# jjshoots/PyFlyt

Measured on AMD Instinct MI355X. Metric: env-steps/sec (whole node), QuadX-Hover batch=65536 per GPU, higher is better.
Workload: dtype f32

## Files before the change

pyflyt_amd/csrc/quadx_fast.hpp:

```cpp
#pragma once
#include <cstdlib>
#include <cstring>
#include <type_traits>

#include "../../include/pyflyt_amd.h"
#include "uav_device.hpp"
#include "uav_vehicles.hpp"
#include "quadx_control_d.hpp"
#include "shared_world.hpp"
#include "policy_mlp.hpp"

namespace pf {

struct QuadK {
  float dt, half_dt, gravity_z, vmax, inv_mass;
  float I[3], iI[3];
  float use_gyro;
  float bound_radius;
  float bound_radius0, slop;
  float margin;
  float brk, rd;
  float c_erp;
  int32_t c_all8;
  float box_h[3], plane_xy, plane_z;
// ... 1006 lines not shown
  const int op = FIXED ? (int)OP_STEP : op_arg;
  const uint8_t* const mask = FIXED ? nullptr : mask_arg;
  const int k_autoreset = FIXED ? (int)PF_AUTORESET_NEXT_STEP : K.autoreset;
  const int k_step_ratio = FIXED ? kQuadFixedRatio<TASK> : K.env_step_ratio;
  const bool k_quat = FIXED || K.angle_repr != 0;
  const bool k_sparse = !FIXED && K.task_sparse != 0;
  constexpr bool REKEY = TASK == PF_TASK_HOVER || TASK == PF_TASK_WAYPOINTS;
  constexpr bool SPARE = REKEY && !MODES && !SHARED && NOISE != PF_NOISE_INJECT;
  typedef QuadSpare Sp;
  constexpr bool GIVEN = ROLL == 2;
  constexpr int kMaxD = 13 + 4 + 4 + 16;
  constexpr int kSettleMax = 24;
  __shared__ __attribute__((aligned(16))) float tile_all[kQuadWPB * LPW * kMaxD];
  __shared__ __attribute__((aligned(16))) float sxi_all[kQuadWPB * 64 * kSettleMax];
  __shared__ int spos_all[kQuadWPB * 64];
  __shared__ float wpose_all[SHARED ? kQuadWPB * 64 * 8 : 1];
  __shared__ float wvel_all[SHARED ? kQuadWPB * 64 * kPairVelStride : 1];
  __shared__ uint32_t sctr_all[kQuadWPB * 64];
  __shared__ __attribute__((aligned(16))) float splds_all[(ROLLOUT && SPARE) ? kQuadWPB * 64 * 20 : 4];
  const int wid = kQuadWPB > 1 ? (int)(threadIdx.x >> 6) : 0;
  const int tid = kQuadWPB > 1 ? (int)(threadIdx.x & 63u) : (int)threadIdx.x;
  float* const tile = tile_all + wid * (LPW * kMaxD);
  float* const sxi = sxi_all + wid * (64 * kSettleMax);
  int* const spos = spos_all + wid * 64;
  uint32_t* const sctr = sctr_all + wid * 64;
  float* const wpose = wpose_all + (SHARED ? wid * 64 * 8 : 0);
  const int apw = SHARED ? K.apw : 1;
  const int wave_base = (blockIdx.x * kQuadWPB + wid) * LPW;
  if (kQuadWPB > 1 && wave_base >= n) return;
  const int lane = wave_base + tid;
  const bool valid = (tid < LPW) && (lane < n);
  const size_t li = valid ? (size_t)lane : (size_t)(n - 1);
  const size_t N = (size_t)n;
  const float4* Sin = reinterpret_cast<const float4*>(B.state);
  float4* Sout = reinterpret_cast<float4*>(B.state);
#ifdef PF_PHASE_TRACE
  unsigned long long pf_ts[kPhaseStamps];
  pf_ts[11] = __builtin_amdgcn_s_memrealtime();
#endif
  PF_STAMP(0);

  QuadHot V;
  constexpr bool DSTATE = MODES && !SHARED;
  QuadStateD SD;
  static_assert(LPW * kMaxD >= kContactSlotFloats, "the contact solver's LDS regions alias the observation tile: at least one worst-case region");
  V.cws = (lds_fptr)tile;
  V.cws_floats = LPW * kMaxD;
  if (SHARED) { V.wpose_ = wpose; V.wvel_ = wvel_all + wid * 64 * kPairVelStride; V.rec_ = tile; V.wtid = tid; V.wA = apw; }
  QuadCascT<typename std::conditional<DSTATE, double, float>::type> C;
  const pf_params_kptr Pk = uniform_params(Pfull);
  constexpr bool CALM = CR && !SHARED && !MODES && NOISE != PF_NOISE_INJECT;
  QuadKV KV{};
  if (CALM) KV = quadkv_from(K);
  float tgt[4][3];
  float new_dist, old_dist;
  int step_count, flags, n_left;
  uint32_t rng_ctr;
  f8 zn;
  uint32_t call0 = 0u;
  uint32_t rkw = 0u;
  bool sp_dirty = false;
  uint32_t reset_key_now = 0u;
  Sp spv{};
  float* const splds = splds_all + ((ROLLOUT && SPARE) ? (wid * 64 + tid) * 20 : 0);
  float4 a_pre = float4{0.f, 0.f, 0.f, 0.f};
  const float4 f4z = float4{0.f, 0.f, 0.f, 0.f};
  float4 cm0 = f4z, cm1 = f4z, cm2 = f4z, cm3 = f4z, cm4 = f4z, cm5 = f4z, cm6 = f4z, cm7 = f4z, cm8 = f4z, cm9 = f4z;
  {
    float4 gi = Sin[6 * N + li];
    float4 g0 = Sin[0 * N + li], g1 = Sin[1 * N + li], g2 = Sin[2 * N + li], g3 = Sin[3 * N + li], g4 = Sin[4 * N + li],
           g5 = Sin[5 * N + li];
    float4 gs7 = float4{0.f, 0.f, 0.f, 0.f};
    if (SPARE) gs7 = Sin[7 * N + li];
    if (SPARE) {
      typedef const uint32_t __attribute__((address_space(1))) * gu32ptr;
      uintptr_t ca = reinterpret_cast<uintptr_t>(launch_ctr + kCtrStride * blockIdx.x);
      asm volatile("" : "+v"(ca));
      call0 = *reinterpret_cast<gu32ptr>(ca);
    }
    if (ROLL == 0 && op == OP_STEP) a_pre = reinterpret_cast<const float4*>(B.actions)[li];
    float4 dl0 = float4{0.f, 0.f, 0.f, 0.f}, dl1 = dl0, dl2 = dl0, dl3 = dl0;
    float4 dl4 = dl0, dl5 = dl0;
    if (DSTATE) { dl0 = Sin[16 * N + li]; dl1 = Sin[17 * N + li]; dl2 = Sin[18 * N + li]; dl3 = Sin[19 * N + li]; dl4 = Sin[20 * N + li]; dl5 = Sin[21 * N + li]; }
    if (MODES) {
      cm0 = Sin[7 * N + li]; cm1 = Sin[8 * N + li]; cm2 = Sin[9 * N + li]; cm3 = Sin[10 * N + li]; cm4 = Sin[11 * N + li];
      if (DSTATE) { cm5 = Sin[22 * N + li]; cm6 = Sin[23 * N + li]; cm7 = Sin[24 * N + li]; cm8 = Sin[25 * N + li]; cm9 = Sin[26 * N + li]; }
    }
    if (CR && blockIdx.x < kRareTextPrefetchBlocks) rare_text_prefetch(tid);
    rng_ctr = (uint32_t)__float_as_int(gi.z);
    PF_STAMP(1);
    if (REKEY) {
      const bool in11 = MODES && K.mode > 0;
      const bool need_sp = SPARE || ROLLOUT || in11 || op == OP_RESET || k_autoreset == PF_AUTORESET_SAME_STEP ||
                           (__float_as_int(gi.y) & (PF_F_TERMINATED | PF_F_TRUNCATED)) != 0;
      if (need_sp) {
        const float4 gk = SPARE ? gs7 : (in11 ? cm4 : (MODES ? cm0 : Sin[(size_t)7 * N + li]));
        rkw = (uint32_t)__float_as_int(in11 ? gk.z : gk.w);
        if (SPARE && op == OP_RESET && mask == nullptr) rkw &= ~kSpareValid;
        if (SPARE) {
          spv.z = gk.x; spv.vz = gk.y; spv.thr = gk.z;
          if constexpr (ROLL == 3) {
            float4* r4 = reinterpret_cast<float4*>(splds);
            r4[0] = float4{spv.z, spv.vz, spv.thr, 0.0f};
            if (TASK == PF_TASK_WAYPOINTS) { r4[1] = Sin[8 * N + li]; r4[2] = Sin[9 * N + li]; r4[3] = Sin[10 * N + li]; r4[4] = Sin[11 * N + li]; }
          } else {
          if (TASK == PF_TASK_WAYPOINTS) { spv.t[0] = Sin[8 * N + li]; spv.t[1] = Sin[9 * N + li]; spv.t[2] = Sin[10 * N + li]; spv.t[3] = Sin[11 * N + li]; }
          if (ROLLOUT) {
            float4* r4 = reinterpret_cast<float4*>(splds);
            r4[0] = float4{spv.z, spv.vz, spv.thr, 0.0f};
            if (TASK == PF_TASK_WAYPOINTS) { r4[1] = spv.t[0]; r4[2] = spv.t[1]; r4[3] = spv.t[2]; r4[4] = spv.t[3]; }
          }
          }
        }
      }
    }
    if (NOISE == PF_NOISE_PHILOX) {
      if (op == OP_STEP) zn = normal8(philox4x32(K.seed_lo, K.seed_hi, (uint32_t)(lane0 + li), rng_ctr, 0u, 0u));
    }
    PF_STAMP(2);
    V.p = v3{g0.x, g0.y, g0.z}; new_dist = g0.w;
    V.q = quat{g1.x, g1.y, g1.z, g1.w};
    V.set_wv(v3{g2.w, g3.x, g3.y}, v3{g2.x, g2.y, g2.z});
    V.t01 = f2{g3.z, g3.w}; V.t23 = f2{g4.x, g4.y};
    V.I[0] = g4.z; V.I[1] = g4.w; V.I[2] = g5.x;
    V.E[0] = g5.y; V.E[1] = g5.z; V.E[2] = g5.w;
    if (DSTATE) {
      SD.p[0] = (double)g0.x + (double)dl0.x; SD.p[1] = (double)g0.y + (double)dl0.y; SD.p[2] = (double)g0.z + (double)dl0.z;
      SD.q[0] = (double)g1.x + (double)dl0.w; SD.q[1] = (double)g1.y + (double)dl1.x; SD.q[2] = (double)g1.z + (double)dl1.y; SD.q[3] = (double)g1.w + (double)dl1.z;
      SD.v[0] = (double)g2.x + (double)dl1.w; SD.v[1] = (double)g2.y + (double)dl2.x; SD.v[2] = (double)g2.z + (double)dl2.y;
      SD.w[0] = (double)g2.w + (double)dl2.z; SD.w[1] = (double)g3.x + (double)dl2.w; SD.w[2] = (double)g3.y + (double)dl3.x;
      SD.rI[0] = (double)g4.z + (double)dl4.x; SD.rI[1] = (double)g4.w + (double)dl4.y; SD.rI[2] = (double)g5.x + (double)dl4.z;
      SD.rE[0] = (double)g5.y + (double)dl4.w; SD.rE[1] = (double)g5.z + (double)dl5.x; SD.rE[2] = (double)g5.w + (double)dl5.y;
      SD.thr[0] = (double)g3.z + (double)dl3.y; SD.thr[1] = (double)g3.w + (double)dl3.z; SD.thr[2] = (double)g4.x + (double)dl3.w; SD.thr[3] = (double)g4.y + (double)dl5.z;
#pragma unroll
      for (int k = 0; k < 4; ++k) SD.pwm[k] = 0.05;
      SD.derive();
    }
    step_count = __float_as_int(gi.x); flags = __float_as_int(gi.y);
    n_left = __float_as_int(gi.w);
    if (TASK == PF_TASK_WAYPOINTS || TASK == PF_TASK_MA_HOVER) {
      float4 a = Sin[12 * N + li], b = Sin[13 * N + li], c = Sin[14 * N + li];
      tgt[0][0] = a.x; tgt[0][1] = a.y; tgt[0][2] = a.z; tgt[1][0] = a.w;
      tgt[1][1] = b.x; tgt[1][2] = b.y; tgt[2][0] = b.z; tgt[2][1] = b.w;
      tgt[2][2] = c.x; tgt[3][0] = c.y; tgt[3][1] = c.z; tgt[3][2] = c.w;
    }
  }
  old_dist = new_dist;
  if (MODES && K.mode > 0) {
    C.unpack(cm0, cm1, cm2, cm3, cm4, false);
    if constexpr (DSTATE) C.unpack(cm5, cm6, cm7, cm8, cm9, true);
  } else C.zero();
  float4 ma_past = float4{0.f, 0.f, 0.f, 0.f};
  if (TASK == PF_TASK_MA_HOVER) ma_past = Sin[15 * N + li];
  const bool kYaw = (TASK == PF_TASK_WAYPOINTS) && K.use_yaw != 0;
  float ytg[4] = {0.f, 0.f, 0.f, 0.f};
  float yaw_err0 = 0.0f;
  if (kYaw) { float4 y = Sin[15 * N + li]; ytg[0] = y.x; ytg[1] = y.y; ytg[2] = y.z; ytg[3] = y.w; }
  auto yaw_now = [&]() {
    if (__builtin_fabsf(V.R.m20) >= 0.99999f) return euler_from_quat(V.q).z;
    return fast_atan2(V.R.m10, V.R.m00);
  };
  auto wrap_pi = [](float e) {
    e = e > kPi ? e - 2.0f * kPi : e;
    return e < -kPi ? e + 2.0f * kPi : e;
  };
  V.contact_now = (flags & PF_F_CONTACT) != 0;
  V.contact_step = false;
  V.derive();
#ifdef PF_PHASE_TRACE
  asm volatile("" ::"v"(V.wb.x), "v"(V.vb.z));
#endif
  PF_STAMP(3);
  bool term = (flags & PF_F_TERMINATED) != 0, trunc = (flags & PF_F_TRUNCATED) != 0;

  bool active;
  if (op == OP_RESET) active = (mask == nullptr) || (mask[li] != 0);
  else active = true;
  active = active && valid;
  if (SHARED && op == OP_RESET) active = widen_to_world(active, tid, apw) && valid;

  float act0 = 0.f, act1 = 0.f, act2 = 0.f, act3 = 0.f;
  float reward = 0.0f;
  bool pop_pending = false;
  bool was_reset = false;
  const int D = (k_quat ? 13 : 12) + 8 + (TASK == PF_TASK_WAYPOINTS ? (kYaw ? 4 : 3) * K.num_targets : (TASK == PF_TASK_MA_HOVER ? 3 : 0));
  const int settle_ticks = K.settle_steps * 2;

  auto pop_target = [&]() {
#pragma unroll
    for (int k = 0; k < 3; ++k)
#pragma unroll
      for (int c = 0; c < 3; ++c) tgt[k][c] = tgt[k + 1][c];
    ytg[0] = ytg[1]; ytg[1] = ytg[2]; ytg[2] = ytg[3];
    n_left -= 1;
  };
  auto lds_sync = [&]() { lds_sync_wave(); };
  const bool coop_targets = (TASK == PF_TASK_WAYPOINTS) && !((NOISE == PF_NOISE_INJECT) && (B.u_targets != nullptr));
  auto prepare_reset_draws = [&](const bool reset_now, const uint32_t key) {
    const bool want_noise = NOISE == PF_NOISE_PHILOX;
    if (!want_noise && !coop_targets) return;
    const unsigned long long m = __ballot(reset_now);
    if (m == 0ull) return;
    const int r = __popcll(m);
    uint32_t seed_lo = K.seed_lo, seed_hi = K.seed_hi;
    asm volatile("" : "+s"(seed_lo), "+s"(seed_hi));
    if (reset_now) {
      spos[__popcll(m & ((1ull << tid) - 1ull))] = tid;
      sctr[tid] = key;
    }
    lds_sync();
    const int ncall = want_noise ? (settle_ticks + 7) >> 3 : 0;
    const int nt = K.num_targets, ntc = coop_targets ? (kYaw ? 4 : 3) : 0;
    const int per = ncall + ntc;
    float* const U = tile;
    float* const TG = tile + 64 * 16;
    for (int base = 0; base < r * per; base += 64) {
      const int j = base + tid;
      if (j < r * per) {
        const int which = j / per, c = j - which * per;
        const int src = spos[which];
// ... 218 lines not shown
            phi = B.u_targets[(size_t)(nt + i) * N + li] * (0.5f / kPi);
            dist = B.u_targets[(size_t)(2 * nt + i) * N + li];
          } else {
            theta = u(i);
            phi = u(nt + i);
            dist = fmaf(K.dome09m1, u(2 * nt + i), 1.0f);
          }
          float st, ct, sph, cph;
          sincos_turns(theta, st, ct);
          sincos_turns(phi, sph, cph);
          float zz = __builtin_fabsf(dist * cph);
          tgt[i][0] = dist * sph * ct; tgt[i][1] = dist * sph * st; tgt[i][2] = zz > K.min_height ? zz : K.min_height;
        }
      }
      }
      float dx = tgt[0][0] - V.p.x, dy = tgt[0][1] - V.p.y, dz = tgt[0][2] - V.p.z;
      old_dist = INFINITY;
      new_dist = fsqrt(fmaf(dx, dx, fmaf(dy, dy, dz * dz)));
      if (kYaw) yaw_err0 = __builtin_fabsf(wrap_pi(ytg[0] - yaw_now()));
    }
    rng_ctr += 1;
    if (REKEY) { rkw = rng_ctr & ~kSpareValid; sp_dirty = true; }
    was_reset = true;
  };
  auto make_spare = [&](const bool me, const uint32_t key, Sp& out) {
    prepare_reset_draws(me, key);
    if (me) {
      float z = K.start_pos[2], vz = 0.f, thr = 0.f, pw = 0.05f;
      settle_run(z, vz, thr, pw);
      out.z = z; out.vz = vz; out.thr = thr;
      if (TASK == PF_TASK_WAYPOINTS) {
        const float4* t4 = reinterpret_cast<const float4*>(tile + 64 * 16 + tid * 16);
#pragma unroll
        for (int i = 0; i < 4; ++i) out.t[i] = t4[i];
      }
    }
  };
  auto spare_get = [&]() -> Sp {
    if (!ROLLOUT) return spv;
    Sp x;
    const float4* r4 = reinterpret_cast<const float4*>(splds);
    const float4 a0 = r4[0];
    x.z = a0.x; x.vz = a0.y; x.thr = a0.z;
    if (TASK == PF_TASK_WAYPOINTS) { x.t[0] = r4[1]; x.t[1] = r4[2]; x.t[2] = r4[3]; x.t[3] = r4[4]; }
    return x;
  };
  auto spare_put = [&](const Sp& x) {
    if (!ROLLOUT) { spv = x; return; }
    float4* r4 = reinterpret_cast<float4*>(splds);
    r4[0] = float4{x.z, x.vz, x.thr, 0.0f};
    if (TASK == PF_TASK_WAYPOINTS) { r4[1] = x.t[0]; r4[2] = x.t[1]; r4[3] = x.t[2]; r4[4] = x.t[3]; }
  };
  auto do_resets = [&](const bool r) {
    const bool have = SPARE && r && (rkw & kSpareValid) != 0u;
    reset_key_now = REKEY ? (rkw & ~kSpareValid) : rng_ctr;
    prepare_reset_draws(r && !have, reset_key_now);
    if (!MODES || __any(r)) {
      if (r) {
        if (SPARE && __builtin_expect(have, 1)) reset_lane(true, spare_get());
        else reset_lane(false, Sp{});
      }
    }
  };
  auto refill_spares = [&](const bool now) {
    if (!SPARE || !now) return;
    const bool want = active && (rkw & kSpareValid) == 0u;
    if (!__any(want)) return;
    Sp g{};
    make_spare(want, rkw & ~kSpareValid, g);
    if (want) { spare_put(g); rkw |= kSpareValid; sp_dirty = true; }
  };
  auto write_obs_row = [&]() {
    float* row = tile + tid * D;
    float sarg = -V.R.m20;
    quat qe;
    v3 rpy;
    const float obs_yaw = kYaw ? yaw_now() : 0.0f;
    if (__builtin_fabsf(sarg) >= 0.99999f) {
      rpy = euler_from_quat(V.q);
      qe = quat_from_euler(rpy);
    } else {
      float ar = V.R.m21, br = V.R.m22;
      float ay = V.R.m10, by = V.R.m00;
      float hr = frsq(fmaf(ar, ar, br * br)), hy = frsq(fmaf(ay, ay, by * by));
      float cr, sr, cp, sp, cy, sy;
      half_angle(br * hr, ar * hr, cr, sr);
      half_angle(fsqrt((1.0f - sarg) * (1.0f + sarg)), sarg, cp, sp);
      half_angle(by * hy, ay * hy, cy, sy);
      quat t = quat_from_half_angles(cr, sr, cp, sp, cy, sy);
      float inv = frsq(fmaf(t.x, t.x, fmaf(t.y, t.y, fmaf(t.z, t.z, t.w * t.w))));
      qe = quat{t.x * inv, t.y * inv, t.z * inv, t.w * inv};
      if (!k_quat) rpy = v3{fast_atan2(ar, br), fast_asin(sarg), fast_atan2(ay, by)};
    }
    int k = 0;
    row[k++] = V.wb.x; row[k++] = V.wb.y; row[k++] = V.wb.z;
    if (k_quat) { row[k++] = qe.x; row[k++] = qe.y; row[k++] = qe.z; row[k++] = qe.w; }
    else { row[k++] = rpy.x; row[k++] = rpy.y; row[k++] = rpy.z; }
    row[k++] = V.vb.x; row[k++] = V.vb.y; row[k++] = V.vb.z;
    row[k++] = V.p.x; row[k++] = V.p.y; row[k++] = V.p.z;
    if (TASK == PF_TASK_MA_HOVER) {
      row[k++] = V.t01.x; row[k++] = V.t01.y; row[k++] = V.t23.x; row[k++] = V.t23.y;
      row[k++] = ma_past.x; row[k++] = ma_past.y; row[k++] = ma_past.z; row[k++] = ma_past.w;
      row[k++] = tgt[0][0]; row[k++] = tgt[0][1]; row[k++] = tgt[0][2];
    } else {
      row[k++] = act0; row[k++] = act1; row[k++] = act2; row[k++] = act3;
      row[k++] = V.t01.x; row[k++] = V.t01.y; row[k++] = V.t23.x; row[k++] = V.t23.y;
    }
// ... 13 lines not shown
  const bool wave_all = __all(active || !valid);

  const int KS = ROLLOUT ? k_steps : 1;
  float4 a_nxt = float4{0.f, 0.f, 0.f, 0.f};
  if (GIVEN) a_nxt = reinterpret_cast<const float4*>(B.actions)[li];
  lds_fptr polh = nullptr;
  pol_cptr polP = nullptr;
  if constexpr (ROLL == 3) {
    __shared__ __attribute__((aligned(16))) float polh_all[kQuadWPB * kPolH * 64];
    polh = (lds_fptr)(polh_all + wid * (kPolH * 64) + tid);
    polP = pol_uniform(PK.packed);
  }
  auto policy_action = [&](const int slot) -> float4 {
    const float4 m = policy_mean(PK, polP, (lds_fptr)(tile + tid * D), D, polh);
    float4 a = m;
    if (PK.has_std) {
      const f8 e = normal8(philox4x32(K.seed_lo, K.seed_hi, (uint32_t)(lane0 + li), step0 + (uint32_t)slot, 0u, 4u));
      a = float4{fmaf(polP[kPolStd + 0], e.v[0], m.x), fmaf(polP[kPolStd + 1], e.v[1], m.y), fmaf(polP[kPolStd + 2], e.v[2], m.z),
                 fmaf(polP[kPolStd + 3], e.v[3], m.w)};
    }
    if (active) {
      const size_t o = 4 * ((size_t)slot * N + li);
      if (PK.mean_out != nullptr) {
        float* mo = PK.mean_out + o;
        __builtin_nontemporal_store(m.x, mo + 0); __builtin_nontemporal_store(m.y, mo + 1);
        __builtin_nontemporal_store(m.z, mo + 2); __builtin_nontemporal_store(m.w, mo + 3);
      }
      if (B.actions_out != nullptr) {
        float* ao = B.actions_out + o;
        __builtin_nontemporal_store(a.x, ao + 0); __builtin_nontemporal_store(a.y, ao + 1);
        __builtin_nontemporal_store(a.z, ao + 2); __builtin_nontemporal_store(a.w, ao + 3);
      }
    }
    return a;
  };
  if constexpr (ROLL == 3) {
    if (active) {
      const float* o0 = PK.obs0 + li * (size_t)D;
      float* row = tile + tid * D;
      for (int k = 0; k < D; ++k) row[k] = o0[k];
    }
    lds_sync_wave();
    a_nxt = policy_action(0);
    lds_sync_wave();
  }
  for (int it = 0; it < KS; ++it) {
  const size_t toff = ROLLOUT ? (size_t)it * N : (size_t)0;
  bool do_reset;
  if (op == OP_RESET) do_reset = active;
  else do_reset = (k_autoreset == PF_AUTORESET_NEXT_STEP) && (term || trunc) && active;
  act0 = act1 = act2 = act3 = 0.f;
  reward = 0.0f;
  was_reset = false;
  do_resets(do_reset);
  const uint32_t call0_u = SPARE ? (uint32_t)__builtin_amdgcn_readfirstlane((int)call0) : 0u;
  refill_spares(op == OP_RESET || ((call0_u + (uint32_t)it) % kSpareEvery) == kSpareEvery - 1u);
  PF_STAMP(4);

  const bool stepping = active && !was_reset && op == OP_STEP;
  float sp0 = 0.f, sp1 = 0.f, sp2 = 0.f, sp3 = 0.f;
  float4 a_roll = float4{0.f, 0.f, 0.f, 0.f};
  if (ROLLOUT) {
    if (GIVEN) {
      a_roll = a_nxt;
      if (it + 1 < KS) a_nxt = reinterpret_cast<const float4*>(B.actions)[toff + N + li];
    } else if constexpr (ROLL == 3) {
      a_roll = a_nxt;
    } else {
      f4 u = uniform4(philox4x32(K.seed_lo, K.seed_hi, (uint32_t)(lane0 + li), step0 + (uint32_t)it, 0u, 3u));
      a_roll = float4{fmaf(K.act_span[0], u.a, K.act_lo[0]), fmaf(K.act_span[1], u.b, K.act_lo[1]),
                      fmaf(K.act_span[2], u.c, K.act_lo[2]), fmaf(K.act_span[3], u.d, K.act_lo[3])};
    }
    if (!GIVEN && ROLL != 3 && B.actions_out != nullptr && active) {
      float* ao = B.actions_out + 4 * (toff + li);
      __builtin_nontemporal_store(a_roll.x, ao + 0); __builtin_nontemporal_store(a_roll.y, ao + 1);
      __builtin_nontemporal_store(a_roll.z, ao + 2); __builtin_nontemporal_store(a_roll.w, ao + 3);
    }
  }
  if (stepping) {
    const float4 a = ROLLOUT ? a_roll : a_pre;
    act0 = a.x; act1 = a.y; act2 = a.z; act3 = a.w;
    sp0 = a.x; sp1 = a.y; sp2 = a.z; sp3 = a.w;
    reward = -0.1f;
    if (TASK == PF_TASK_MA_HOVER) {
      ma_past = float4{tgt[2][1], tgt[2][2], tgt[3][0], tgt[3][1]};
      tgt[2][1] = a.x; tgt[2][2] = a.y; tgt[3][0] = a.z; tgt[3][1] = a.w;
      reward = 0.0f;
      term = false; trunc = false;
    }
  }
  bool go = stepping && !(term || trunc);
  constexpr bool NF = WPS == 1 && (TASK == PF_TASK_HOVER || TASK == PF_TASK_MA_HOVER || (TASK == PF_TASK_WAYPOINTS && ROLLOUT));
  constexpr bool NFX = NF && CALM;
  bool calm = false;
  auto sink_within = [&](const float T, const float TT) {
    const float tm = __builtin_fmaxf(__builtin_fmaxf(__builtin_fabsf(V.t01.x), __builtin_fabsf(V.t01.y)), __builtin_fmaxf(__builtin_fabsf(V.t23.x), __builtin_fabsf(V.t23.y)));
    const float a_nd = fmaf(K.calm_kt, __builtin_fmaxf(tm * tm, K.calm_t2), __builtin_fabsf(K.gravity_z));
    const float u = fsqrt(fmaf(V.wvx.y, V.wvx.y, fmaf(V.wvy.y, V.wvy.y, V.wvz.y * V.wvz.y))) + a_nd * T;
    return fmaf(__builtin_fabsf(V.wvz.y), T, fmaf(K.calm_c, u * u, a_nd) * TT);
  };
  if (CALM && K.calm_on) {
    calm = __all(!go || ((!NF || !V.contact_now) && V.p.z - fmaf(sink_within(K.calm_T, K.calm_TT), 1.01f, 1e-3f) > K.bound_radius));
#ifdef PF_PHASE_TRACE
    if (!calm && tid == 0) trace_add(&g_calm_trace[0], 1ull);
#endif
  }
  for (int s = 0; s < k_step_ratio; ++s) {
    if (!__any(go)) break;
    bool calm_s = calm;
    if (CALM && K.calm_on && !calm) {
      calm_s = __all(!go || ((!NF || !V.contact_now) && V.p.z - fmaf(sink_within(K.calm_T2, K.calm_TT2), 1.01f, 1e-3f) > K.bound_radius));
#ifdef PF_PHASE_TRACE
      if (!calm_s && tid == 0) trace_add(&g_calm_trace[1], 1ull);
#endif
    }
    if (go) {
      float xi0, xi1;
      if (NOISE == PF_NOISE_PHILOX) { xi0 = 4.0f + pick8(zn, (uint32_t)(2 * s)); xi1 = 4.0f + pick8(zn, (uint32_t)(2 * s + 1)); }
      else if (NOISE == PF_NOISE_INJECT) { xi0 = B.xi[(size_t)(2 * s) * N + li]; xi1 = B.xi[(size_t)(2 * s + 1) * N + li]; }
      else { xi0 = 0.f; xi1 = 0.f; }
      V.contact_step = false;
      V.template control<MODES>(K, Pk, C, sp0, sp1, sp2, sp3, DSTATE ? &SD : nullptr);
      if (SHARED) {
        quad_world_exchange(V, wpose, tid, apw, K);
        V.template tick<CR, true>(K, K, xi0, Pfull);
        quad_world_exchange(V, wpose, tid, apw, K);
        V.template tick<CR, true>(K, K, xi1, Pfull);
        V.peer_contact = false;
      } else if (CALM && __builtin_expect(calm_s, 1)) {
        V.template tick<false, false, QuadKV, false, true, NF>(KV, K, xi0, Pfull);
        V.template tick<false, false, QuadKV, false, true, NF>(KV, K, xi1, Pfull);
      } else if (CALM && WPS == 1) {
        V.template tick<CR, false, QuadKV, true>(KV, K, xi0, Pfull);
        V.template tick<CR, false, QuadKV, true>(KV, K, xi1, Pfull);
        if (NFX && V.contact_step) {
          if (TASK == PF_TASK_MA_HOVER) reward -= 100.0f; else reward = -100.0f;
          flags |= PF_F_INFO_COLLISION; term = true;
        }
      } else if (DSTATE) {
        V.template tick_d<CR, WPS == 1>(SD, K, xi0, Pfull);
        V.template tick_d<CR, WPS == 1>(SD, K, xi1, Pfull);
      } else {
        V.template tick<CR, false, QuadK, WPS == 1, !(TASK == PF_TASK_HOVER && WPS == 2)>(K, K, xi0, Pfull);
        V.template tick<CR, false, QuadK, WPS == 1, !(TASK == PF_TASK_HOVER && WPS == 2)>(K, K, xi1, Pfull);
      }
      if (TASK == PF_TASK_WAYPOINTS) {
        if (pop_pending) { pop_target(); pop_pending = false; }
        float dx = tgt[0][0] - V.p.x, dy = tgt[0][1] - V.p.y, dz = tgt[0][2] - V.p.z;
        old_dist = new_dist;
        new_dist = fsqrt(fmaf(dx, dx, fmaf(dy, dy, dz * dz)));
        if (kYaw) yaw_err0 = __builtin_fabsf(wrap_pi(ytg[0] - yaw_now()));
      }
      if (step_count > K.max_steps) trunc = true;
      if (TASK == PF_TASK_MA_HOVER) {
        if (!NFX && V.contact_step) { reward -= 100.0f; flags |= PF_F_INFO_COLLISION; term = true; }
        if (dot(V.p, V.p) > K.dome2) { reward -= 100.0f; flags |= PF_F_INFO_OOB; term = true; }
        if (!k_sparse) {
          float dx = V.p.x - tgt[0][0], dy = V.p.y - tgt[0][1], dz = V.p.z - tgt[0][2];
          float lin = fsqrt(fmaf(dx, dx, fmaf(dy, dy, dz * dz)));
          float sarg = -V.R.m20;
          bool gim = __builtin_fabsf(sarg) >= 0.99999f;
          float roll = gim ? 0.0f : fast_atan2(V.R.m21, V.R.m22);
          float pitch = gim ? __builtin_copysignf(0.5f * kPi, sarg) : fast_asin(sarg);
          float ang = fsqrt(fmaf(roll, roll, pitch * pitch));
          reward -= fmaf(ang, 0.1f, lin);
          reward += 1.0f;
        }
      } else {
      if (!NFX && V.contact_step) { reward = -100.0f; flags |= PF_F_INFO_COLLISION; term = true; }
      if (dot(V.p, V.p) > K.dome2) { reward = -100.0f; flags |= PF_F_INFO_OOB; term = true; }
      }
      if (TASK == PF_TASK_HOVER) {
        if (!k_sparse) {
          float dz = V.p.z - 1.0f;
          float lin = fsqrt(fmaf(V.p.x, V.p.x, fmaf(V.p.y, V.p.y, dz * dz)));
          float sarg = -V.R.m20;
          bool gim = __builtin_fabsf(sarg) >= 0.99999f;
          float roll = gim ? 0.0f : fast_atan2(V.R.m21, V.R.m22);
          float pitch = gim ? __builtin_copysignf(0.5f * kPi, sarg) : fast_asin(sarg);
          float ang = fsqrt(fmaf(roll, roll, pitch * pitch));
          reward = fmaf(-0.01f * V.wb.z, V.wb.z, reward);
          reward -= lin + ang;
          reward += 1.0f;
        }
      } else if (TASK == PF_TASK_WAYPOINTS) {
        if (!k_sparse) {
          float progress = (isinf(old_dist + new_dist)) ? 0.0f : old_dist - new_dist;
          reward += __builtin_fmaxf(3.0f * progress, 0.0f);
          reward = fmaf(K.wp_dist_reward, frcp(new_dist), reward);
          reward = fmaf(-K.wp_yaw_penalty * V.wb.z, V.wb.z, reward);
        }
        if (new_dist < K.goal_reach && (!kYaw || yaw_err0 < K.goal_angle)) {
          reward = 100.0f;
          pop_pending = true;
          if (n_left - 1 == 0) { trunc = true; flags |= PF_F_INFO_COMPLETE; }
        }
      }
      if (TASK != PF_TASK_MA_HOVER) go = !(term || trunc);
    }
  }
  PF_STAMP(5);
  const float out_reward = stepping ? reward : 0.0f;
  const bool out_term = stepping && term, out_trunc = stepping && trunc;
  if (stepping) {
    step_count += 1; rng_ctr += 1;
    const float chk = ((V.p.x + V.p.y) + (V.p.z + V.q.x)) + ((V.q.y + V.q.z) + (V.q.w + V.wvx.y)) + ((V.wvy.y + V.wvz.y) + (V.wvx.x + V.wvy.x)) +
                      ((V.wvz.x + V.t01.x) + (V.t01.y + V.t23.x)) + ((V.t23.y + V.I[0]) + (V.I[1] + V.I[2]));
    if (!(__builtin_fabsf(chk) < INFINITY)) flags |= PF_F_NONFINITE;
  }

  if (k_autoreset == PF_AUTORESET_SAME_STEP) {
    const bool same = stepping && (term || trunc);
    if (__any(same)) {
      if (B.final_obs != nullptr) {
        if (active) write_obs_row();
        flush_obs_tile(tile, B.final_obs + toff * D, D, LPW, n, wave_base, tid, wave_all, active);
      }
      if (B.final_info != nullptr && same) {
        B.final_info[2 * (toff + li) + 0] = done_flags(flags, term, trunc, V.contact_now);
        B.final_info[2 * (toff + li) + 1] = n_left - (pop_pending ? 1 : 0);
      }
      do_resets(same);
    }
  }

  PF_STAMP(6);
  if (active) write_obs_row();
  PF_STAMP(7);
  flush_obs_tile(tile, B.obs + toff * D, D, LPW, n, wave_base, tid, wave_all, active);
  PF_STAMP(8);
  if (active) {
    if (pop_pending) { pop_target(); pop_pending = false; }
    flags = done_flags(flags, term, trunc, V.contact_now);
    if (op == OP_STEP) {
      B.reward[toff + li] = out_reward;
      B.terminated[toff + li] = out_term ? 1 : 0;
      B.truncated[toff + li] = out_trunc ? 1 : 0;
    }
  }
  if (ROLLOUT && DSTATE) {
    SD.through_hilo();
    if constexpr (DSTATE) C.through_hilo();
  }
  if (ROLLOUT && NOISE == PF_NOISE_PHILOX && it + 1 < KS)
    zn = normal8(philox4x32(K.seed_lo, K.seed_hi, (uint32_t)(lane0 + li), rng_ctr, 0u, 0u));
  if constexpr (ROLL == 3) {
    if (it + 1 < KS) a_nxt = policy_action(it + 1);
  }
  }
  if (SPARE && op == OP_STEP && tid == 0) launch_ctr[kCtrStride * blockIdx.x] = call0 + (uint32_t)KS;
  if (active) {
// ... 56 lines not shown
```

pyflyt_amd/csrc/uav_device.hpp:

```cpp
#pragma once
#include <hip/hip_runtime.h>
#include <stdint.h>

#define PF_DEV __device__ __forceinline__

namespace pf {

constexpr float kPi = 3.14159265358979323846f;

struct v3 {
  float x, y, z;
};
PF_DEV v3 mk3(float x, float y, float z) { return v3{x, y, z}; }
PF_DEV v3 operator+(v3 a, v3 b) { return v3{a.x + b.x, a.y + b.y, a.z + b.z}; }
PF_DEV v3 operator-(v3 a, v3 b) { return v3{a.x - b.x, a.y - b.y, a.z - b.z}; }
PF_DEV v3 operator*(float s, v3 a) { return v3{s * a.x, s * a.y, s * a.z}; }
PF_DEV float dot(v3 a, v3 b) { return fmaf(a.x, b.x, fmaf(a.y, b.y, a.z * b.z)); }
PF_DEV v3 cross(v3 a, v3 b) {
  return v3{fmaf(a.y, b.z, -(a.z * b.y)), fmaf(a.z, b.x, -(a.x * b.z)), fmaf(a.x, b.y, -(a.y * b.x))};
}
PF_DEV float clampf(float x, float lo, float hi) { return __builtin_fminf(__builtin_fmaxf(x, lo), hi); }
PF_DEV float sq_signed(float x) { return x * __builtin_fabsf(x); }

struct quat {
// ... 28 lines not shown
  float sqx = q.x * q.x, sqy = q.y * q.y, sqz = q.z * q.z, squ = q.w * q.w;
  float sarg = -2.0f * (q.x * q.z - q.w * q.y) / (sqx + sqy + sqz + squ);
  v3 e;
  if (sarg <= -0.99999f) {
    e = v3{0.0f, -0.5f * kPi, 2.0f * atan2f(q.x, -q.y)};
  } else if (sarg >= 0.99999f) {
    e = v3{0.0f, 0.5f * kPi, 2.0f * atan2f(-q.x, q.y)};
  } else {
    e.x = atan2f(2.0f * (q.y * q.z + q.w * q.x), squ - sqx - sqy + sqz);
    e.y = asinf(sarg);
    e.z = atan2f(2.0f * (q.x * q.y + q.w * q.z), squ + sqx - sqy - sqz);
  }
  return e;
}
PF_DEV quat quat_from_euler(v3 e) {
  float sr, cr, sp, cp, sy, cy;
  sincosf(0.5f * e.x, &sr, &cr);
  sincosf(0.5f * e.y, &sp, &cp);
  sincosf(0.5f * e.z, &sy, &cy);
  quat q{sr * cp * cy - cr * sp * sy, cr * sp * cy + sr * cp * sy, cr * cp * sy - sr * sp * cy, cr * cp * cy + sr * sp * sy};
  float inv = rsqrtf(fmaf(q.x, q.x, fmaf(q.y, q.y, fmaf(q.z, q.z, q.w * q.w))));
  return quat{q.x * inv, q.y * inv, q.z * inv, q.w * inv};
}

typedef float f2 __attribute__((ext_vector_type(2)));
PF_DEV f2 fma2(f2 a, f2 b, f2 c) { return __builtin_elementwise_fma(a, b, c); }
PF_DEV f2 sp2(float x) { return f2{x, x}; }
PF_DEV float frcp(float x) { return __builtin_amdgcn_rcpf(x); }
PF_DEV float frsq(float x) { return __builtin_amdgcn_rsqf(x); }
PF_DEV float fsqrt(float x) { return __builtin_amdgcn_sqrtf(x); }
PF_DEV float med3(float x, float lo, float hi) { return __builtin_amdgcn_fmed3f(x, lo, hi); }
PF_DEV float fast_atan2(float y, float x) {
  float ax = __builtin_fabsf(x), ay = __builtin_fabsf(y);
  float mx = __builtin_fmaxf(ax, ay), mn = __builtin_fminf(ax, ay);
  float t = mn * frcp(mx);
  t = (mx == 0.0f) ? 0.0f : t;
  float s = t * t;
  float p = fmaf(s, 0.0029035410843789577f, -0.016282962635159492f);
  p = fmaf(s, p, 0.04303929582238197f);
  p = fmaf(s, p, -0.07533670216798782f);
  p = fmaf(s, p, 0.10654674470424652f);
  p = fmaf(s, p, -0.14207133650779724f);
  p = fmaf(s, p, 0.19993053376674652f);
  p = fmaf(s, p, -0.3333309292793274f);
  p = fmaf(s, p, 1.0f);
  float r = p * t;
  r = (ay > ax) ? (0.5f * kPi - r) : r;
  r = (x < 0.0f) ? (kPi - r) : r;
  return __builtin_copysignf(r, y);
}
PF_DEV float fast_asin(float x) {
  return fast_atan2(x, fsqrt(__builtin_fmaxf((1.0f - x) * (1.0f + x), 0.0f)));
}
PF_DEV quat quat_from_half_angles(float cr, float sr, float cp, float sp, float cy, float sy) {
  const float a = sr * cp, b = cr * sp, c = cr * cp, d = sr * sp;
  return quat{fmaf(a, cy, -(b * sy)), fmaf(b, cy, a * sy), fmaf(c, sy, -(d * cy)), fmaf(c, cy, d * sy)};
}
PF_DEV void half_angle(float c, float s, float& ch, float& sh) {
  const float a = fsqrt(0.5f * (1.0f + __builtin_fabsf(c)));
  const float b = 0.5f * s * frcp(a);
  const bool pos = c >= 0.0f;
  ch = pos ? a : __builtin_fabsf(b);
  sh = pos ? b : __builtin_copysignf(a, s);
}

PF_DEV void sincos_small(float x, float& sn, float& cs) {
  const float t = x * x;
  sn = x * fmaf(t, fmaf(t, fmaf(t, fmaf(t, fmaf(t, -2.5052108e-8f, 2.7557319e-6f), -1.9841270e-4f), 8.3333333e-3f), -1.6666667e-1f), 1.0f);
  cs = fmaf(t, fmaf(t, fmaf(t, fmaf(t, fmaf(t, fmaf(t, 2.0876757e-9f, -2.7557319e-7f), 2.4801587e-5f), -1.3888889e-3f), 4.1666667e-2f), -0.5f), 1.0f);
}
PF_DEV void sincos_turns(float u, float& sn, float& cs) {
  const float k = __builtin_rintf(4.0f * u);
  const float r = (2.0f * kPi) * fmaf(k, -0.25f, u);
  float s, c;
  sincos_small(r, s, c);
  const int q = (int)k & 3;
  const bool odd = (q & 1) != 0;
  const float a = odd ? c : s, b = odd ? s : c;
  sn = (q & 2) ? -a : a;
  cs = (q == 1 || q == 2) ? -b : b;
}
PF_DEV v3 euler_from_quat_fast(quat q) {
  float sqx = q.x * q.x, sqy = q.y * q.y, sqz = q.z * q.z, squ = q.w * q.w;
  float sarg = -2.0f * (q.x * q.z - q.w * q.y) * frcp(sqx + sqy + sqz + squ);
  if (sarg <= -0.99999f) return v3{0.0f, -0.5f * kPi, 2.0f * fast_atan2(q.x, -q.y)};
  if (sarg >= 0.99999f) return v3{0.0f, 0.5f * kPi, 2.0f * fast_atan2(-q.x, q.y)};
  return v3{fast_atan2(2.0f * (q.y * q.z + q.w * q.x), squ - sqx - sqy + sqz), fast_asin(sarg),
            fast_atan2(2.0f * (q.x * q.y + q.w * q.z), squ + sqx - sqy - sqz)};
}
PF_DEV quat canon_quat(quat q) {
  float sqx = q.x * q.x, sqy = q.y * q.y, sqz = q.z * q.z, squ = q.w * q.w;
  float sarg = -2.0f * (q.x * q.z - q.w * q.y) * frcp(sqx + sqy + sqz + squ);
  if (__builtin_fabsf(sarg) >= 0.99999f) return quat_from_euler(euler_from_quat(q));
  float ar = 2.0f * (q.y * q.z + q.w * q.x), br = squ - sqx - sqy + sqz;
  float ay = 2.0f * (q.x * q.y + q.w * q.z), by = squ + sqx - sqy - sqz;
  float hr = frsq(fmaf(ar, ar, br * br)), hy = frsq(fmaf(ay, ay, by * by));
  float cr, sr, cp, sp, cy, sy;
  half_angle(br * hr, ar * hr, cr, sr);
  half_angle(fsqrt((1.0f - sarg) * (1.0f + sarg)), sarg, cp, sp);
  half_angle(by * hy, ay * hy, cy, sy);
  quat t = quat_from_half_angles(cr, sr, cp, sp, cy, sy);
  float inv = frsq(fmaf(t.x, t.x, fmaf(t.y, t.y, fmaf(t.z, t.z, t.w * t.w))));
  return quat{t.x * inv, t.y * inv, t.z * inv, t.w * inv};
}

PF_DEV quat quat_integrate(quat q, v3 w, float half_dt) {
// ... 59 lines not shown
    sep |= (__builtin_fabsf(t[i]) - rad > 0.0f);
  }
#pragma unroll
  for (int j = 0; j < 3; ++j) {
    float proj = t[0] * Rm[0][j] + t[1] * Rm[1][j] + t[2] * Rm[2][j];
    float rad = ha[j] + Q[0][j] * hb[0] + Q[1][j] * hb[1] + Q[2][j] * hb[2];
    sep |= (__builtin_fabsf(proj) - rad > 0.0f);
  }
#pragma unroll
  for (int i = 0; i < 3; ++i) {
    const int i1 = (i + 1) % 3, i2 = (i + 2) % 3;
#pragma unroll
    for (int j = 0; j < 3; ++j) {
      const int j1 = (j + 1) % 3, j2 = (j + 2) % 3;
      float expr1 = t[i2] * Rm[i1][j] - t[i1] * Rm[i2][j];
      float rad = hb[i1] * (Q[i2][j] + 1e-5f) + hb[i2] * (Q[i1][j] + 1e-5f) + ha[j1] * (Q[i][j2] + 1e-5f) +
                  ha[j2] * (Q[i][j1] + 1e-5f);
      sep |= (__builtin_fabsf(expr1) - rad > 2.220446e-16f);
    }
  }
  return !sep;
}

PF_DEV bool cyl_overlaps_aabb(v3 c, const m3& R, float r, float hl, v3 cb, const float hb[3]) {
  const float ax[3] = {R.m02, R.m12, R.m22};
  const float t[3] = {c.x - cb.x, c.y - cb.y, c.z - cb.z};
  bool sep = false;
#pragma unroll
  for (int k = 0; k < 3; ++k) {
    float s2 = __builtin_fmaxf(1.0f - ax[k] * ax[k], 0.0f);
    float ext = hl * __builtin_fabsf(ax[k]) + r * __builtin_sqrtf(s2);
    sep |= (__builtin_fabsf(t[k]) - (hb[k] + ext) > 0.0f);
  }
  return !sep;
}

#ifndef PF_PHILOX_ROUNDS
#define PF_PHILOX_ROUNDS 10
#endif
struct u32x4 {
  uint32_t a, b, c, d;
};
PF_DEV u32x4 philox4x32(uint32_t k0, uint32_t k1, uint32_t c0, uint32_t c1, uint32_t c2, uint32_t c3) {
#pragma unroll
  for (int r = 0; r < PF_PHILOX_ROUNDS; ++r) {
    uint32_t hi0 = __umulhi(0xD2511F53u, c0), lo0 = 0xD2511F53u * c0;
    uint32_t hi1 = __umulhi(0xCD9E8D57u, c2), lo1 = 0xCD9E8D57u * c2;
    uint32_t n0 = hi1 ^ c1 ^ k0, n2 = hi0 ^ c3 ^ k1;
    c0 = n0; c1 = lo1; c2 = n2; c3 = lo0;
    k0 += 0x9E3779B9u; k1 += 0xBB67AE85u;
  }
  return u32x4{c0, c1, c2, c3};
}
PF_DEV float u01(uint32_t x) { return ((float)(x >> 9) + 0.5f) * (1.0f / 8388608.0f); }
struct f4 {
  float a, b, c, d;
};
PF_DEV f4 uniform4(u32x4 r) { return f4{u01(r.a), u01(r.b), u01(r.c), u01(r.d)}; }
struct f8 {
  float v[8];
};
PF_DEV void bm16(uint32_t w, float& z0, float& z1) {
  float u1 = ((float)(w & 0xFFFFu) + 0.5f) * (1.0f / 65536.0f);
  float u2 = (float)(w >> 16) * (1.0f / 65536.0f);
  float rad = __builtin_amdgcn_sqrtf(-1.3862943611198906f * __builtin_amdgcn_logf(u1));
  z0 = rad * __builtin_amdgcn_cosf(u2);
  z1 = rad * __builtin_amdgcn_sinf(u2);
}
PF_DEV f8 normal8(u32x4 r) {
  f8 z;
  bm16(r.a, z.v[0], z.v[1]);
  bm16(r.b, z.v[2], z.v[3]);
  bm16(r.c, z.v[4], z.v[5]);
  bm16(r.d, z.v[6], z.v[7]);
  return z;
}
PF_DEV float pick8(const f8& z, uint32_t i) {
  float a = (i & 1u) ? z.v[1] : z.v[0], b = (i & 1u) ? z.v[3] : z.v[2];
  float c = (i & 1u) ? z.v[5] : z.v[4], d = (i & 1u) ? z.v[7] : z.v[6];
  float lo = (i & 2u) ? b : a, hi = (i & 2u) ? d : c;
  return (i & 4u) ? hi : lo;
}
PF_DEV float pick4(f4 v, uint32_t i) {
  float lo = (i & 1u) ? v.b : v.a, hi = (i & 1u) ? v.d : v.c;
  return (i & 2u) ? hi : lo;
}

}
```

Baseline: 7.239 billion.

## Specialize fixed hover path: split Philox, paired atan2, select-based reset, unrolled substeps

For the fixed-ratio hover specialization, several independent micro-optimizations are added. The first Philox rounds that depend only on the lane index are hoisted ahead of the counter load. Roll and pitch atan2 now go through a paired packed-float polynomial with register-pinned constants. Spare-state resets become branchless selects applied before derive, replacing the reset routine. The physics substep loop is fully unrolled with compile-time step index and calm flag. Together these aim to cut ALU work and divergence, at the cost of more register pressure and code size.

```diff
diff --git a/pyflyt_amd/csrc/quadx_fast.hpp b/pyflyt_amd/csrc/quadx_fast.hpp
--- a/pyflyt_amd/csrc/quadx_fast.hpp
+++ b/pyflyt_amd/csrc/quadx_fast.hpp
@@ -1082,6 +1082,8 @@
   constexpr bool CALM = CR && !SHARED && !MODES && NOISE != PF_NOISE_INJECT;
   QuadKV KV{};
   if (CALM) KV = quadkv_from(K);
+  constexpr bool PKREW = FIXED && WPS == 1 && TASK == PF_TASK_HOVER;
+  Atan2C AC{};
   float tgt[4][3];
   float new_dist, old_dist;
   int step_count, flags, n_left;
@@ -1116,6 +1118,13 @@
       cm0 = Sin[7 * N + li]; cm1 = Sin[8 * N + li]; cm2 = Sin[9 * N + li]; cm3 = Sin[10 * N + li]; cm4 = Sin[11 * N + li];
       if (DSTATE) { cm5 = Sin[22 * N + li]; cm6 = Sin[23 * N + li]; cm7 = Sin[24 * N + li]; cm8 = Sin[25 * N + li]; cm9 = Sin[26 * N + li]; }
     }
+    constexpr bool PHX = FIXED && WPS == 1 && NOISE == PF_NOISE_PHILOX;
+    PhiloxPre zpre{};
+    if constexpr (PHX) {
+      zpre = philox4x32_pre(K.seed_hi, (uint32_t)(lane0 + li));
+      asm volatile("" : "+v"(zpre.lo0), "+v"(zpre.hi1), "+v"(zpre.lo1));
+    }
+    if constexpr (PKREW) AC = atan2_consts();
     if (CR && blockIdx.x < kRareTextPrefetchBlocks) rare_text_prefetch(tid);
     rng_ctr = (uint32_t)__float_as_int(gi.z);
     PF_STAMP(1);
@@ -1145,7 +1154,8 @@
       }
     }
     if (NOISE == PF_NOISE_PHILOX) {
-      if (op == OP_STEP) zn = normal8(philox4x32(K.seed_lo, K.seed_hi, (uint32_t)(lane0 + li), rng_ctr, 0u, 0u));
+      if constexpr (PHX) zn = normal8(philox4x32_post(K.seed_lo, K.seed_hi, zpre, rng_ctr));
+      else if (op == OP_STEP) zn = normal8(philox4x32(K.seed_lo, K.seed_hi, (uint32_t)(lane0 + li), rng_ctr, 0u, 0u));
     }
     PF_STAMP(2);
     V.p = v3{g0.x, g0.y, g0.z}; new_dist = g0.w;
@@ -1196,6 +1206,21 @@
   };
   V.contact_now = (flags & PF_F_CONTACT) != 0;
   V.contact_step = false;
+  constexpr bool SEL = FIXED && SPARE && WPS == 1 && TASK == PF_TASK_HOVER;
+  bool sel = false;
+  if constexpr (SEL) {
+    sel = valid && (flags & (PF_F_TERMINATED | PF_F_TRUNCATED)) != 0 && (rkw & kSpareValid) != 0u;
+    V.p = v3{sel ? K.start_pos[0] : V.p.x, sel ? K.start_pos[1] : V.p.y, sel ? spv.z : V.p.z};
+    V.q = quat{sel ? K.start_quat[0] : V.q.x, sel ? K.start_quat[1] : V.q.y, sel ? K.start_quat[2] : V.q.z, sel ? K.start_quat[3] : V.q.w};
+    V.wvx = f2{sel ? 0.0f : V.wvx.x, sel ? 0.0f : V.wvx.y};
+    V.wvy = f2{sel ? 0.0f : V.wvy.x, sel ? 0.0f : V.wvy.y};
+    V.wvz = f2{sel ? 0.0f : V.wvz.x, sel ? spv.vz : V.wvz.y};
+    V.t01 = f2{sel ? spv.thr : V.t01.x, sel ? spv.thr : V.t01.y};
+    V.t23 = f2{sel ? spv.thr : V.t23.x, sel ? spv.thr : V.t23.y};
+#pragma unroll
+    for (int k = 0; k < 3; ++k) { V.I[k] = sel ? 0.0f : V.I[k]; V.E[k] = sel ? 0.0f : V.E[k]; }
+    V.contact_now = V.contact_now && !sel;
+  }
   V.derive();
 #ifdef PF_PHASE_TRACE
   asm volatile("" ::"v"(V.wb.x), "v"(V.vb.z));
@@ -1520,7 +1545,7 @@
     if (TASK == PF_TASK_WAYPOINTS) { r4[1] = x.t[0]; r4[2] = x.t[1]; r4[3] = x.t[2]; r4[4] = x.t[3]; }
   };
   auto do_resets = [&](const bool r) {
-    const bool have = SPARE && r && (rkw & kSpareValid) != 0u;
+    const bool have = SPARE && !SEL && r && (rkw & kSpareValid) != 0u;
     reset_key_now = REKEY ? (rkw & ~kSpareValid) : rng_ctr;
     prepare_reset_draws(r && !have, reset_key_now);
     if (!MODES || __any(r)) {
@@ -1640,7 +1665,15 @@
   act0 = act1 = act2 = act3 = 0.f;
   reward = 0.0f;
   was_reset = false;
-  do_resets(do_reset);
+  if constexpr (SEL) {
+    step_count = sel ? 0 : step_count; flags = sel ? 0 : flags;
+    term = term && !sel; trunc = trunc && !sel;
+    rng_ctr += sel ? 1u : 0u;
+    rkw = sel ? (rng_ctr & ~kSpareValid) : rkw;
+    sp_dirty = sp_dirty || sel;
+    was_reset = sel;
+  }
+  do_resets(SEL ? (do_reset && !sel) : do_reset);
   const uint32_t call0_u = SPARE ? (uint32_t)__builtin_amdgcn_readfirstlane((int)call0) : 0u;
   refill_spares(op == OP_RESET || ((call0_u + (uint32_t)it) % kSpareEvery) == kSpareEvery - 1u);
   PF_STAMP(4);
@@ -1693,8 +1726,9 @@
     if (!calm && tid == 0) trace_add(&g_calm_trace[0], 1ull);
 #endif
   }
-  for (int s = 0; s < k_step_ratio; ++s) {
-    if (!__any(go)) break;
+  auto aviary_step = [&](const auto s_c, const auto calm_c) __attribute__((always_inline)) {
+    const int s = s_c;
+    const bool calm = calm_c;
     bool calm_s = calm;
     if (CALM && K.calm_on && !calm) {
       calm_s = __all(!go || ((!NF || !V.contact_now) && V.p.z - fmaf(sink_within(K.calm_T2, K.calm_TT2), 1.01f, 1e-3f) > K.bound_radius));
@@ -1764,8 +1798,15 @@
           float lin = fsqrt(fmaf(V.p.x, V.p.x, fmaf(V.p.y, V.p.y, dz * dz)));
           float sarg = -V.R.m20;
           bool gim = __builtin_fabsf(sarg) >= 0.99999f;
-          float roll = gim ? 0.0f : fast_atan2(V.R.m21, V.R.m22);
-          float pitch = gim ? __builtin_copysignf(0.5f * kPi, sarg) : fast_asin(sarg);
+          float roll, pitch;
+          if constexpr (PKREW) {
+            const f2 rp = fast_atan2_x2(f2{V.R.m21, sarg}, f2{V.R.m22, fsqrt(__builtin_fmaxf((1.0f - sarg) * (1.0f + sarg), 0.0f))}, AC);
+            roll = gim ? 0.0f : rp.x;
+            pitch = gim ? __builtin_copysignf(0.5f * kPi, sarg) : rp.y;
+          } else {
+            roll = gim ? 0.0f : fast_atan2(V.R.m21, V.R.m22);
+            pitch = gim ? __builtin_copysignf(0.5f * kPi, sarg) : fast_asin(sarg);
+          }
           float ang = fsqrt(fmaf(roll, roll, pitch * pitch));
           reward = fmaf(-0.01f * V.wb.z, V.wb.z, reward);
           reward -= lin + ang;
@@ -1785,6 +1826,29 @@
         }
       }
       if (TASK != PF_TASK_MA_HOVER) go = !(term || trunc);
+    }
+  };
+  constexpr bool STRAIGHT = FIXED && CALM && WPS == 1 && TASK == PF_TASK_HOVER;
+  if (STRAIGHT && calm) {
+    if constexpr (STRAIGHT) {
+      typedef std::integral_constant<bool, true> calm_t;
+      do {
+        if (!__any(go)) break;
+        aviary_step(std::integral_constant<int, 0>{}, calm_t{});
+        if (!__any(go)) break;
+        aviary_step(std::integral_constant<int, 1>{}, calm_t{});
+        if (!__any(go)) break;
+        aviary_step(std::integral_constant<int, 2>{}, calm_t{});
+        if constexpr (kQuadFixedRatio<TASK> == 4) {
+          if (!__any(go)) break;
+          aviary_step(std::integral_constant<int, 3>{}, calm_t{});
+        }
+      } while (false);
+    }
+  } else {
+    for (int s = 0; s < k_step_ratio; ++s) {
+      if (!__any(go)) break;
+      aviary_step(s, calm);
     }
   }
   PF_STAMP(5);
diff --git a/pyflyt_amd/csrc/uav_device.hpp b/pyflyt_amd/csrc/uav_device.hpp
--- a/pyflyt_amd/csrc/uav_device.hpp
+++ b/pyflyt_amd/csrc/uav_device.hpp
@@ -104,6 +104,40 @@
 PF_DEV float fast_asin(float x) {
   return fast_atan2(x, fsqrt(__builtin_fmaxf((1.0f - x) * (1.0f + x), 0.0f)));
 }
+struct Atan2C {
+  float c[8];
+  float half_pi, pi;
+};
+PF_DEV Atan2C atan2_consts() {
+  Atan2C k{{0.0029035410843789577f, -0.016282962635159492f, 0.04303929582238197f, -0.07533670216798782f, 0.10654674470424652f,
+            -0.14207133650779724f, 0.19993053376674652f, -0.3333309292793274f}, 0.5f * kPi, kPi};
+#pragma unroll
+  for (int i = 0; i < 8; ++i) asm volatile("" : "+v"(k.c[i]));
+  asm volatile("" : "+v"(k.half_pi), "+v"(k.pi));
+  return k;
+}
+PF_DEV f2 fast_atan2_x2(f2 y, f2 x, const Atan2C& k) {
+  const float ax0 = __builtin_fabsf(x.x), ay0 = __builtin_fabsf(y.x), ax1 = __builtin_fabsf(x.y), ay1 = __builtin_fabsf(y.y);
+  const float mx0 = __builtin_fmaxf(ax0, ay0), mn0 = __builtin_fminf(ax0, ay0);
+  const float mx1 = __builtin_fmaxf(ax1, ay1), mn1 = __builtin_fminf(ax1, ay1);
+  f2 t = f2{mn0, mn1} * f2{frcp(mx0), frcp(mx1)};
+  t = f2{(mx0 == 0.0f) ? 0.0f : t.x, (mx1 == 0.0f) ? 0.0f : t.y};
+  const f2 s = t * t;
+  f2 p = fma2(s, sp2(k.c[0]), sp2(k.c[1]));
+  p = fma2(s, p, sp2(k.c[2]));
+  p = fma2(s, p, sp2(k.c[3]));
+  p = fma2(s, p, sp2(k.c[4]));
+  p = fma2(s, p, sp2(k.c[5]));
+  p = fma2(s, p, sp2(k.c[6]));
+  p = fma2(s, p, sp2(k.c[7]));
+  p = fma2(s, p, sp2(1.0f));
+  f2 r = p * t;
+  const f2 h = sp2(k.half_pi) - r;
+  r = f2{(ay0 > ax0) ? h.x : r.x, (ay1 > ax1) ? h.y : r.y};
+  const f2 g = sp2(k.pi) - r;
+  r = f2{(x.x < 0.0f) ? g.x : r.x, (x.y < 0.0f) ? g.y : r.y};
+  return f2{__builtin_copysignf(r.x, y.x), __builtin_copysignf(r.y, y.y)};
+}
 PF_DEV quat quat_from_half_angles(float cr, float sr, float cp, float sp, float cy, float sy) {
   const float a = sr * cp, b = cr * sp, c = cr * cp, d = sr * sp;
   return quat{fmaf(a, cy, -(b * sy)), fmaf(b, cy, a * sy), fmaf(c, sy, -(d * cy)), fmaf(c, cy, d * sy)};
@@ -269,6 +303,30 @@
   }
   return u32x4{c0, c1, c2, c3};
 }
+struct PhiloxPre {
+  uint32_t lo0, hi1, lo1;
+};
+PF_DEV PhiloxPre philox4x32_pre(uint32_t k1, uint32_t c0) {
+  const uint32_t c2 = __umulhi(0xD2511F53u, c0) ^ k1;
+  return PhiloxPre{0xD2511F53u * c0, __umulhi(0xCD9E8D57u, c2), 0xCD9E8D57u * c2};
+}
+PF_DEV u32x4 philox4x32_post(uint32_t k0, uint32_t k1, PhiloxPre h, uint32_t c1) {
+  static_assert(PF_PHILOX_ROUNDS >= 2, "the split takes the first two rounds apart");
+  const uint32_t a = c1 ^ k0;
+  k0 += 0x9E3779B9u; k1 += 0xBB67AE85u;
+  const uint32_t hi0 = __umulhi(0xD2511F53u, a), lo0 = 0xD2511F53u * a;
+  uint32_t c0 = h.hi1 ^ k0, c1n = h.lo1, c2 = hi0 ^ h.lo0 ^ k1, c3 = lo0;
+  k0 += 0x9E3779B9u; k1 += 0xBB67AE85u;
+#pragma unroll
+  for (int r = 2; r < PF_PHILOX_ROUNDS; ++r) {
+    uint32_t h0 = __umulhi(0xD2511F53u, c0), l0 = 0xD2511F53u * c0;
+    uint32_t h1 = __umulhi(0xCD9E8D57u, c2), l1 = 0xCD9E8D57u * c2;
+    uint32_t n0 = h1 ^ c1n ^ k0, n2 = h0 ^ c3 ^ k1;
+    c0 = n0; c1n = l1; c2 = n2; c3 = l0;
+    k0 += 0x9E3779B9u; k1 += 0xBB67AE85u;
+  }
+  return u32x4{c0, c1n, c2, c3};
+}
 PF_DEV float u01(uint32_t x) { return ((float)(x >> 9) + 0.5f) * (1.0f / 8388608.0f); }
 struct f4 {
   float a, b, c, d;
```

After: 7.666 billion (median of 6 runs). 1.06x the previous value.
